# mahfuzalhasan/WaveFormer

Hardware: AMD Instinct MI355X
Metric: 128³×4 volumes/sec fwd (1/2/4/8 MI355X) + Dice Δ vs reference (higher is better)
Workload: dtype bf16x3

## Files before the change

### include/waveformer_hip.h

```cpp
#ifndef WAVEFORMER_HIP_H
#define WAVEFORMER_HIP_H

#include <stdint.h>

#ifdef __cplusplus
extern "C" {
#endif

#define WF_ABI_VERSION 21

enum { WF_PREC_BF16 = 0, WF_PREC_BF16X3 = 1, WF_PREC_FP16 = 2 };

enum {
  WF_OK = 0,
  WF_E_SHAPE = -1,
  WF_E_NULLPTR = -2,
  WF_E_LAUNCH = -3
};

int wf_abi_version(void);
const char* wf_last_error(void);


int wf_cast_f32_to_bf16(const float* in, uint16_t* out, int64_t n, void* stream);

int wf_split_f32_to_bf16x2(const float* in, uint16_t* out, int64_t n, void* stream);

int wf_split_f32_to_bf16x2_multi(const int64_t* table_dev, int64_t n, int64_t total,
                                 void* stream);

int wf_cast_f32_to_f16x2(const float* in, uint16_t* out, int64_t n, void* stream);
int wf_cast_f32_to_f16x2_multi(const int64_t* table_dev, int64_t n, int64_t total,
                               void* stream);

int wf_debug_poison_lds(int64_t blocks, int lds_bytes, void* stream);

int wf_patch_embed_fwd(const float* x, const float* w, const float* bias, float* out,
                       int64_t B, int64_t Cin, int64_t Cout, int64_t D, int64_t H, int64_t W,
                       void* stream);
int wf_patch_embed_ll_fwd(const float* x, const float* w, const float* bias, float* out,
                          const float* ln_w, const float* ln_b, float ln_eps, float* ll,
                          int64_t B, int64_t Cin, int64_t Cout, int64_t D, int64_t H, int64_t W,
// ... 159 lines not shown
int wf_window_attention_levels_fused(const int64_t* dhw, int nlev, int64_t B, int64_t C,
                                     int64_t heads, int precision);

int wf_msfuse_fwd(const float* const* src, const int64_t* src_dhw, int nsrc,
                  const float* shortcut, const float* branch_scale, float* out, float* stats,
                  float ln_eps, int64_t B, int64_t C, int64_t D, int64_t H, int64_t W,
                  void* stream);

int64_t wf_ccf_ffn_workspace_bytes(int64_t B, int64_t C, int64_t hidden, int64_t D, int64_t H,
                                   int64_t W, int precision);
int wf_ccf_ffn_fwd(const float* xh, const float* stats, const float* n2_w, const float* n2_b,
                   const uint16_t* pw_bf16x2, const float* pw_b, const float* ln1_w,
                   const float* ln1_b, float eps1, const float* dw_w, const float* dw_b,
                   const float* ln2_w, const float* ln2_b, float eps2,
                   const uint16_t* fc_bf16x2, const float* fc_b, const float* branch_scale,
                   float* out, void* workspace,
                   int64_t B, int64_t C, int64_t hidden, int64_t D, int64_t H, int64_t W,
                   int precision, void* stream);
int wf_ccf_ffn_stage(int stage, const float* xh, const float* stats, const float* n2_w,
                     const float* n2_b, const uint16_t* pw_bf16x2, const float* pw_b,
                     const float* ln1_w, const float* ln1_b, float eps1, const float* dw_w,
                     const float* dw_b, const float* ln2_w, const float* ln2_b, float eps2,
                     const uint16_t* fc_bf16x2, const float* fc_b, const float* branch_scale,
                     float* out, void* workspace, int64_t B, int64_t C, int64_t hidden,
                     int64_t D, int64_t H, int64_t W, int precision, void* stream);

int wf_patch_merging_fwd(const float* x, const float* ln_w, const float* ln_b, float eps,
                         const uint16_t* red_bf16x2, int v2, float* out, int64_t B, int64_t C,
                         int64_t D, int64_t H, int64_t W, int precision, void* stream);

int wf_proj_out_fwd(const float* x, float* out, int normalize, float eps, int64_t B,
                    int64_t C, int64_t S, void* stream);
int wf_proj_out_cl_fwd(const float* x, float* out, float eps, int64_t M, int64_t C, void* stream);

int wf_importance_map(int mode, const float* sigma_scale, float* out, int64_t rd, int64_t rh,
                      int64_t rw, void* stream);

int wf_sliding_window_stitch(const float* patches, int64_t world, int64_t slots_per_round,
                             const float* importance_map, const int64_t* starts,
                             const int64_t* nwin, float* out, int64_t B, int64_t C, int64_t D,
                             int64_t H, int64_t W, int64_t rd, int64_t rh, int64_t rw,
                             void* stream);

int wf_sliding_window_stitch_partial(const float* patches, int64_t world, int64_t rank,
                                     const float* importance_map, const int64_t* starts,
                                     const int64_t* nwin, float* out, int64_t B, int64_t C,
                                     int64_t D, int64_t H, int64_t W, int64_t rd, int64_t rh,
                                     int64_t rw, void* stream);
int wf_sliding_window_normalize(const float* num, float* out, int64_t B, int64_t C, int64_t D,
                                int64_t H, int64_t W, void* stream);

int wf_tta_merge(const float* pred, const int* flips, int npass, float* out, int64_t C,
                 int64_t D, int64_t H, int64_t W, void* stream);


int wf_window_attention_fwd_train(const float* x, const float* ln_w, const float* ln_b,
                                  float ln_eps, const uint16_t* wqkv_bf16x2, const float* bqkv,
                                  const float* bias, const uint16_t* wproj_bf16x2,
                                  const float* bproj, float* out, void* workspace, float* lse,
                                  int64_t B, int64_t C, int64_t D1, int64_t H1, int64_t W1,
                                  int64_t ws, int64_t heads, float scale, int precision,
                                  void* stream);

int64_t wf_window_attention_bwd_workspace_bytes(int64_t B, int64_t C, int64_t D1, int64_t H1,
                                                int64_t W1, int64_t ws, int64_t heads);
int wf_window_attention_bwd_core(const float* qkv, const float* o, const float* dout,
// ... 58 lines not shown
```

### waveformer_amd/_lib.py

```python
from __future__ import annotations

import ctypes
import os
import threading

_HERE = os.path.dirname(os.path.abspath(__file__))
LIB_PATH = os.environ.get("WAVEFORMER_HIP_LIB", os.path.join(_HERE, "libwaveformer_hip.so"))

_P = ctypes.c_void_p
_I64 = ctypes.c_int64
_I = ctypes.c_int
_F = ctypes.c_float

SIGNATURES = {
    "wf_abi_version": (_I, []),
    "wf_last_error": (ctypes.c_char_p, []),
    "wf_cast_f32_to_bf16": (_I, [_P, _P, _I64, _P]),
    "wf_split_f32_to_bf16x2": (_I, [_P, _P, _I64, _P]),
    "wf_split_f32_to_bf16x2_multi": (_I, [_P, _I64, _I64, _P]),
    "wf_cast_f32_to_f16x2": (_I, [_P, _P, _I64, _P]),
    "wf_cast_f32_to_f16x2_multi": (_I, [_P, _I64, _I64, _P]),
    "wf_debug_poison_lds": (_I, [_I64, _I, _P]),
    "wf_patch_embed_ll_fwd": (_I, [_P, _P, _P, _P, _P, _P, _F, _P, _I64, _I64, _I64, _I64, _I64,
                                   _I64, _P]),
# ... 40 lines not shown
    "wf_norm_act_bwd_workspace_bytes": (_I64, [_I64, _I64]),
    "wf_norm_act_bwd_cl": (_I, [_P, _I64, _P, _I64, _P, _I64, _P, _P, _I64, _P, _P, _I64, _P, _I64,
                                _I64, _I64, _I64, _F, _P, _P]),
    "wf_hf_refine_workspace_bytes": (_I64, [_I64, _I64]),
    "wf_hf_refine_fwd": (_I, [_P, _I64, _P, _P, _P, _P, _F, _P, _P, _I, _P, _P, _I64, _I64,
                              _I64, _I64, _I64, _P]),
    "wf_norm_act_cl": (_I, [_P, _I64, _P, _P, _I64, _P, _P, _I64, _I64, _I64, _I64, _F, _P]),
    "wf_upsample_trilinear_cl": (_I, [_P, _P, _I64, _I64, _I64, _I64, _I64, _I64, _I64, _I64,
                                      _I, _P]),
    "wf_linear_fwd": (_I, [_P, _P, _P, _P, _I64, _I64, _I64, _I, _I, _P]),
    "wf_window_attention_fwd_table": (_I, [_P, _P, _P, _F, _P, _P, _P, _P, _P, _P, _P,
                                           _I64, _I64, _I64, _I64, _I64, _I64, _I64, _F, _I,
                                           _P]),
    "wf_rel_pos_bias": (_I, [_P, _P, _P, _I64, _I64, _I64, _P]),
    "wf_window_attention_workspace_bytes": (_I64, [_I64, _I64, _I64, _I64, _I64, _I]),
    "wf_window_attention_fwd": (_I, [_P, _P, _P, _F, _P, _P, _P, _P, _P, _P, _P,
                                     _I64, _I64, _I64, _I64, _I64, _I64, _I64, _F, _I, _P]),
    "wf_window_attention_levels_workspace_bytes": (_I64, [_P, _I, _I64, _I64, _I]),
    "wf_window_attention_fwd_levels": (_I, [_P, _P, _I, _P, _P, _P, _P, _P, _P, _P, _I64, _I64,
                                            _I64, _F, _I, _P]),
    "wf_window_attention_fwd_levels_mode": (_I, [_P, _P, _I, _P, _P, _P, _P, _P, _P, _P, _I64,
                                                 _I64, _I64, _F, _I, _P, _I]),
    "wf_window_attention_levels_fused": (_I, [_P, _I, _I64, _I64, _I64, _I]),
    "wf_msfuse_fwd": (_I, [_P, _P, _I, _P, _P, _P, _P, _F, _I64, _I64, _I64, _I64, _I64, _P]),
    "wf_ccf_ffn_workspace_bytes": (_I64, [_I64, _I64, _I64, _I64, _I64, _I64, _I]),
    "wf_ccf_ffn_fwd": (_I, [_P, _P, _P, _P, _P, _P, _P, _P, _F, _P, _P, _P, _P, _F, _P, _P,
                            _P, _P, _P, _I64, _I64, _I64, _I64, _I64, _I64, _I, _P]),
    "wf_ccf_ffn_stage": (_I, [_I, _P, _P, _P, _P, _P, _P, _P, _P, _F, _P, _P, _P, _P, _F, _P,
                              _P, _P, _P, _P, _I64, _I64, _I64, _I64, _I64, _I64, _I, _P]),
    "wf_patch_merging_fwd": (_I, [_P, _P, _P, _F, _P, _I, _P, _I64, _I64, _I64, _I64, _I64,
                                  _I, _P]),
    "wf_proj_out_fwd": (_I, [_P, _P, _I, _F, _I64, _I64, _I64, _P]),
    "wf_proj_out_cl_fwd": (_I, [_P, _P, _F, _I64, _I64, _P]),
    "wf_upsample_dwconv3d_stats_cl": (_I, [_P, _P, _P, _P, _P] + [_I64] * 8 + [_I, _P]),
    "wf_importance_map": (_I, [_I, _P, _P, _I64, _I64, _I64, _P]),
    "wf_sliding_window_stitch": (_I, [_P, _I64, _I64, _P, _P, _P, _P, _I64, _I64, _I64, _I64,
                                      _I64, _I64, _I64, _I64, _P]),
    "wf_tta_merge": (_I, [_P, _P, _I, _P, _I64, _I64, _I64, _I64, _P]),
    "wf_sliding_window_stitch_partial": (_I, [_P, _I64, _I64, _P, _P, _P, _P, _I64, _I64,
                                              _I64, _I64, _I64, _I64, _I64, _I64, _P]),
    "wf_sliding_window_normalize": (_I, [_P, _P, _I64, _I64, _I64, _I64, _I64, _P]),
    "wf_window_attention_fwd_train": (_I, [_P, _P, _P, _F, _P, _P, _P, _P, _P, _P, _P, _P,
                                           _I64, _I64, _I64, _I64, _I64, _I64, _I64, _F, _I,
                                           _P]),
    "wf_window_attention_bwd_workspace_bytes": (_I64, [_I64, _I64, _I64, _I64, _I64, _I64,
                                                       _I64]),
    "wf_window_attention_bwd_core": (_I, [_P, _P, _P, _P, _P, _P, _P, _P, _I64, _I64, _I64,
                                          _I64, _I64, _I64, _I64, _F, _P]),
    "wf_rel_pos_bias_bwd": (_I, [_P, _P, _P, _P, _I64, _I64, _I64, _P]),
    "wf_gemm_tn_workspace_bytes": (_I64, [_I64, _I64, _I64]),
    "wf_gemm_tn": (_I, [_P, _I64, _P, _I64, _P, _I64, _I, _P, _I64, _I64, _I64, _P]),
    "wf_colsum_parts": (_I64, [_I64]),
    "wf_colsum": (_I, [_P, _I64, _I64, _P, _I64, _P, _P, _P]),
    "wf_ln_act_fwd": (_I, [_P, _P, _P, _F, _I, _P, _I64, _I64, _P]),
    "wf_ln_bwd_workspace_floats": (_I64, [_I64, _I64]),
    "wf_ln_act_bwd": (_I, [_P, _P, _P, _F, _I, _P, _P, _P, _P, _P, _P, _I64, _I64, _P]),
    "wf_dwt3d_haar_bwd": (_I, [_P, _P, _P, _I64, _I64, _I64, _I64, _I64, _P]),
    "wf_haar_analysis_ncdhw": (_I, [_P, _I64, _I64, _P, _P, _P, _I64, _I64, _I64, _I64, _I64,
                                    _P]),
    "wf_interp_adjoint_axis": (_I, [_P, _P, _I64, _I64, _I64, _I64, _P, _I64, _P]),
    "wf_interp_adjoint_axis_ac": (_I, [_P, _P, _I64, _I64, _I64, _I64, _P]),
    "wf_dwconv3d_cl": (_I, [_P, _P, _P, _I, _P, _I64, _I64, _I64, _I64, _I64, _P]),
    "wf_dwconv_wgrad_ws_floats": (_I64, [_I64] * 5),
    "wf_dwconv3d_wgrad": (_I, [_P, _P, _P, _P, _I64, _I64, _I64, _I64, _I64, _P]),
    "wf_patch_merging_gather": (_I, [_P, _I, _P, _I64, _I64, _I64, _I64, _I64, _P]),
    "wf_patch_merging_scatter": (_I, [_P, _I, _P, _I64, _I64, _I64, _I64, _I64, _P]),
    "wf_patchify": (_I, [_P, _P, _I, _I64, _I64, _I64, _I64, _I64, _P]),
    "wf_transpose_cs": (_I, [_P, _P, _I64, _I64, _I64, _P]),
}

ABI_VERSION = 21
_lock = threading.Lock()
_lib = None
_err = None


class LibraryMissing(RuntimeError):
    pass


def load(path: str | None = None):
    global _lib, _err
    with _lock:
        if _lib is not None:
            return _lib
        p = path or LIB_PATH
        if not os.path.exists(p):
            _err = f"{p} not found: build it with `python -c 'import __graft_entry__ as g; g.build()'`"
            raise LibraryMissing(_err)
        lib = ctypes.CDLL(p)
        for name, (res, args) in SIGNATURES.items():
            fn = getattr(lib, name)
            fn.restype = res
            fn.argtypes = args
        ver = lib.wf_abi_version()
        if ver != ABI_VERSION:
            raise LibraryMissing(f"{p}: ABI version {ver}, expected {ABI_VERSION} (rebuild)")
        _lib = lib
        return _lib


def call(name: str, *args) -> None:
    lib = load()
    rc = getattr(lib, name)(*args)
# ... 8 lines not shown
```

### waveformer_amd/csrc/ffn.hip

```cpp
#include "kernels.hpp"

namespace wf {

template <typename T>
struct Store4;
template <>
struct Store4<uint16_t> {
  typedef bf16x4 vec;
  static __device__ __forceinline__ f32x4 up(vec u) {
    return f32x4{bf2f((uint16_t)u[0]), bf2f((uint16_t)u[1]), bf2f((uint16_t)u[2]),
                 bf2f((uint16_t)u[3])};
  }
  static __device__ __forceinline__ uint16_t down(float v) { return f2bf(v); }
  static __device__ __forceinline__ vec zero() { return vec{0, 0, 0, 0}; }
  static __device__ __forceinline__ void store4(uint16_t* p, f32x4 v) {
    bf16x4 o;
    o[0] = (short)f2bf(v.x);
    o[1] = (short)f2bf(v.y);
    o[2] = (short)f2bf(v.z);
    o[3] = (short)f2bf(v.w);
    *reinterpret_cast<bf16x4*>(p) = o;
  }
};
template <>
// ... 645 lines not shown
  f.N = (int)C;
  f.K = (int)hidden;
  f.epi = EPI_RESID;
  f.bias = fc_b;
  f.r_x = xh;
  f.r_stats = stats;
  f.r_ln_w = n2_w;
  f.r_ln_b = n2_b;
  f.r_scale = branch_scale;
  f.rows_per_sample = D * H * W;
  f.out = out;
  f.out_bf16 = 0;
  f.ldo = C;
  if (!keep) {
    f.kpart = reinterpret_cast<float*>(h1);
    f.kpart_bytes = one;
  }
  return launch_gemm(f, s, "wf_ccf_ffn_fwd(fc)");
}

extern "C" int wf_ccf_ffn_fwd(const float* xh, const float* stats, const float* n2_w,
                              const float* n2_b, const uint16_t* pw_bf16x2, const float* pw_b,
                              const float* ln1_w, const float* ln1_b, float eps1,
                              const float* dw_w, const float* dw_b, const float* ln2_w,
                              const float* ln2_b, float eps2, const uint16_t* fc_bf16x2,
                              const float* fc_b, const float* branch_scale, float* out,
                              void* workspace, int64_t B, int64_t C, int64_t hidden, int64_t D,
                              int64_t H, int64_t W, int precision, void* stream) {
  return wf_ccf_ffn_stage(0, xh, stats, n2_w, n2_b, pw_bf16x2, pw_b, ln1_w, ln1_b, eps1, dw_w,
                          dw_b, ln2_w, ln2_b, eps2, fc_bf16x2, fc_b, branch_scale, out,
                          workspace, B, C, hidden, D, H, W, precision, stream);
}

extern "C" int wf_patch_merging_fwd(const float* x, const float* ln_w, const float* ln_b,
                                    float eps, const uint16_t* red_bf16x2, int v2, float* out,
                                    int64_t B, int64_t C, int64_t D, int64_t H, int64_t W,
                                    int precision, void* stream) {
  WF_REQUIRE(B >= 1 && C % 8 == 0 && C >= 8, "C must be a positive multiple of 8");
  WF_REQUIRE(D % 2 == 0 && H % 2 == 0 && W % 2 == 0 && D >= 2 && H >= 2 && W >= 2,
             "odd sizes (the F.pad branch, wave_helper.py:180-182) are not supported");
  WF_REQUIRE(valid_prec(precision), "unknown precision");
  WF_REQUIRE_PTR(x);
  WF_REQUIRE_PTR(ln_w);
  WF_REQUIRE_PTR(ln_b);
  WF_REQUIRE_PTR(red_bf16x2);
  WF_REQUIRE_PTR(out);
  GemmArgs g{};
  g.prec = precision;
  g.a_src = x;
  g.a_bf16 = 0;
  g.a_C = (int)C;
  g.a_nseg = 8;
  g.a_map = MAP_MERGE;
  g.merge_code = v2 ? 0x76543210 : 0x71251240;
  g.mB = (int)B;
  g.mD = (int)D;
  g.mH = (int)H;
  g.mW = (int)W;
  g.a_ln = LN_COMPUTE;
  g.a_ln_w = ln_w;
  g.a_ln_b = ln_b;
  g.a_eps = eps;
  g.w = red_bf16x2;
  g.M = B * (D / 2) * (H / 2) * (W / 2);
  g.N = (int)(2 * C);
  g.K = (int)(8 * C);
  g.epi = EPI_STORE;
  g.bias = nullptr;
  g.out = out;
  g.out_bf16 = 0;
  g.ldo = 2 * C;
  if (try_launch_merge_resident(g, (hipStream_t)stream)) return check_launch("wf_patch_merging_fwd");
  return launch_gemm(g, (hipStream_t)stream, "wf_patch_merging_fwd");
}
```

### waveformer_amd/csrc/kernels.hpp

```cpp
#pragma once
#include "wf_common.hpp"

namespace wf {

enum Prec { PREC_BF16 = 0, PREC_SPLIT = 1, PREC_FP16 = 2 };

typedef _Float16 f16x4 __attribute__((ext_vector_type(4)));
typedef _Float16 f16x8 __attribute__((ext_vector_type(8)));
__device__ __forceinline__ uint16_t f2h(float f) { return __builtin_bit_cast(uint16_t, (_Float16)f); }

template <int P>
__device__ __forceinline__ uint16_t op_cvt(float x) {
  if constexpr (P == PREC_FP16) return f2h(x);
  else return f2bf(x);
}
template <int P>
__device__ __forceinline__ short op_lo(float x, uint16_t hi) {
  if constexpr (P == PREC_SPLIT) return (short)f2bf(x - bf2f(hi));
  else return (short)0;
}
template <int P>
__device__ __forceinline__ f32x4 mma32(bf16x8 a, bf16x8 b, f32x4 c) {
  if constexpr (P == PREC_FP16)
    return __builtin_amdgcn_mfma_f32_16x16x32_f16(__builtin_bit_cast(f16x8, a),
// ... 92 lines not shown
  int64_t rows_per_sample;
  float* o_pstats;
  float* kpart;
  int64_t kpart_bytes;
  int ksplit;
  const float* lv_src[WF_MAX_LEVELS];
  int lv_row0[WF_MAX_LEVELS];
  int lv_D[WF_MAX_LEVELS], lv_H[WF_MAX_LEVELS], lv_W[WF_MAX_LEVELS];
};

int launch_gemm(const GemmArgs& g, hipStream_t s, const char* who);
int gemm_kc_pick_nt(const GemmArgs& g);
int launch_instnorm_partial(const float* x, int64_t ldx, int64_t B, int64_t C, int64_t P,
                            double* acc, hipStream_t s);
int try_launch_gemm_rows(const GemmArgs& g, hipStream_t s, bool single_chunk_only);

int launch_attn_core(const void* qkv, const float* bias, void* out, float* lse, int64_t Bw,
                     int N, int heads, int hd, float scale, int prec, hipStream_t s,
                     int table_ws = 0, int64_t pair_windows = -1, const GemmArgs* fused = nullptr);
bool attn_tbl_pair_loop(int64_t wh);

int launch_dwconv_ln_gelu(const void* in, const float* w, const float* b, const float* ln_w,
                          const float* ln_b, float eps, void* out, int B, int Hd, int D, int H,
                          int W, int prec, hipStream_t s);
int launch_dwconv3d(const void* in, const float* w, const float* b, void* out, float* pstats,
                    int B, int Hd, int D, int H, int W, int prec, hipStream_t s,
                    double* cstats = nullptr, const float* ln1_stats = nullptr,
                    const float* ln1_w = nullptr, const float* ln1_b = nullptr, int flip = 0);
int launch_ln_stats_finalize(const float* pstats, int np, int group, float eps, float* out,
                             int64_t M, hipStream_t s);
constexpr int DW_STAT_GROUP = 32;
int try_launch_gemm_kc(const GemmArgs& g, hipStream_t s);
int try_launch_merge_resident(const GemmArgs& g, hipStream_t s);
int try_launch_pw2_resident(const GemmArgs& g, hipStream_t s);
int try_launch_gemm_lnw(const GemmArgs& g, hipStream_t s);
bool gemm_lnw_wide_shape(const GemmArgs& g);

}

#include "ffn_dwfc_common.hpp"
```

### waveformer_amd/csrc/merge.hip

```cpp
#include <algorithm>

#include "gemm_common.hpp"

namespace wf {

constexpr int MR_C = 48;
constexpr int MR_K = 8 * MR_C;
constexpr int MR_N = 2 * MR_C;
constexpr int MR_NT = MR_N / 16;
constexpr int MR_KS = MR_K / 32;
constexpr int MR_KP = MR_K + WF_LDS_KPAD;
constexpr int MR_WAVES = 8;

template <int P>
__global__ __launch_bounds__(64 * MR_WAVES, 1) void merge_res_kernel(GemmArgs g) {
  constexpr bool SPLIT = P == PREC_SPLIT;
  constexpr int NPL = SPLIT ? 2 : 1;
  extern __shared__ __attribute__((aligned(16))) uint16_t Wl[];
  float* lnw = reinterpret_cast<float*>(Wl + NPL * MR_N * MR_KP);
  float* lnb = lnw + MR_K;
  const int tid = threadIdx.x, lane = tid & 63, wid = tid >> 6;
  const int l15 = lane & 15, g4 = lane >> 4;

  constexpr int OCT = MR_K / 8;
  for (int it = tid; it < NPL * MR_N * OCT; it += 64 * MR_WAVES) {
    const int pr = it / OCT, ch = it - pr * OCT;
    *reinterpret_cast<bf16x8*>(Wl + pr * MR_KP + 8 * ch) =
        *reinterpret_cast<const bf16x8*>(g.w + (int64_t)pr * MR_K + 8 * ch);
  }
  for (int i = tid; i < MR_K; i += 64 * MR_WAVES) {
    lnw[i] = g.a_ln_w[i];
    lnb[i] = g.a_ln_b[i];
  }
  __syncthreads();

  const int M = (int)g.M;
  const int ntiles = (M + 15) >> 4;
  const int hd = g.mD >> 1, hh = g.mH >> 1, hw = g.mW >> 1;
  for (int tile = blockIdx.x * MR_WAVES + wid; tile < ntiles; tile += gridDim.x * MR_WAVES) {
    const int row = tile * 16 + l15;
    int r = min(row, M - 1);
    const int x = r % hw;
    r /= hw;
    const int y = r % hh;
    r /= hh;
    const int z = r % hd, b = r / hd;
    const float* src = reinterpret_cast<const float*>(g.a_src) +
                       (int64_t)(((b * g.mD + 2 * z) * g.mH + 2 * y) * g.mW + 2 * x) * MR_C;
    int g4o = g4;
    asm volatile("" : "+v"(g4o));
    int koff[MR_KS];
#pragma unroll
    for (int ks = 0; ks < MR_KS; ++ks) {
      const int k = ks * 32 + 8 * g4o;
      const int seg = k / MR_C, c = k - seg * MR_C;
      const int o = (g.merge_code >> (4 * seg)) & 0xF;
      koff[ks] = ((((o >> 2) & 1) * g.mH + ((o >> 1) & 1)) * g.mW + (o & 1)) * MR_C + c;
    }
    float a[MR_KS][8];
#pragma unroll
    for (int ks = 0; ks < MR_KS; ++ks) {
      const f32x4* p = reinterpret_cast<const f32x4*>(src + koff[ks]);
      const f32x4 u0 = p[0], u1 = p[1];
      a[ks][0] = u0.x; a[ks][1] = u0.y; a[ks][2] = u0.z; a[ks][3] = u0.w;
      a[ks][4] = u1.x; a[ks][5] = u1.y; a[ks][6] = u1.z; a[ks][7] = u1.w;
    }
    const float sh = __shfl(a[0][0], l15, 64);
    float s = 0.f, q = 0.f;
    asm volatile("" : "+v"(q));
#pragma unroll
    for (int ks = 0; ks < MR_KS; ++ks)
#pragma unroll
      for (int j = 0; j < 8; ++j) {
        const float d = a[ks][j] - sh;
        s += d;
        q += d * d;
      }
    s = xsum16(s);
    s = xsum32(s);
    q = xsum16(q);
    q = xsum32(q);
    const float kf = (float)g.K;
    const float ms = s / kf;
    const float mean = sh + ms;
    const float rstd = rsqrtf(fmaxf(q / kf - ms * ms, 0.f) + g.a_eps);

    uint32_t wb = (uint32_t)((l15 * MR_KP + 8 * g4) * 2), lb = (uint32_t)(8 * g4 * 4);
    asm volatile("" : "+v"(wb), "+v"(lb));
    const char* Wb = reinterpret_cast<const char*>(Wl) + wb;
    const char* Lw = reinterpret_cast<const char*>(lnw) + lb;
    const char* Lb = reinterpret_cast<const char*>(lnb) + lb;
    f32x4 acc[MR_NT];
#pragma unroll
    for (int t = 0; t < MR_NT; ++t) acc[t] = f32x4{0.f, 0.f, 0.f, 0.f};
#pragma unroll
    for (int ks = 0; ks < MR_KS; ++ks) {
      __builtin_amdgcn_sched_barrier(0);
      bf16x8 ah, al;
      a_fragment<P>(a[ks], mean, rstd, reinterpret_cast<const float*>(Lw),
                    reinterpret_cast<const float*>(Lb), ks * 32, true, true, false, ah, al);
#pragma unroll
      for (int t = 0; t < MR_NT; ++t) {
        const int wo = (t * 16 * MR_KP + ks * 32) * 2;
        const bf16x8 bh = *reinterpret_cast<const bf16x8*>(Wb + wo);
        const bf16x8 bl = SPLIT ? *reinterpret_cast<const bf16x8*>(Wb + MR_N * MR_KP * 2 + wo) : bh;
        acc[t] = mma3<P>(acc[t], bh, bl, ah, al);
        if (t % 3 == 2) __builtin_amdgcn_sched_barrier(0);
      }
    }
    if (row < M) {
      float* o = reinterpret_cast<float*>(g.out) + (int64_t)row * g.ldo + 4 * g4;
#pragma unroll
      for (int t = 0; t < MR_NT; ++t) *reinterpret_cast<f32x4*>(o + 16 * t) = acc[t];
    }
  }
}

int try_launch_merge_resident(const GemmArgs& g, hipStream_t s) {
  static const bool off = getenv("WF_MERGE_RES") != nullptr && getenv("WF_MERGE_RES")[0] == '0';
  if (off || g.a_map != MAP_MERGE || g.a_C != MR_C || g.K != MR_K || g.N != MR_N ||
      g.a_ln != LN_COMPUTE || g.a_bf16 || g.out_bf16 || g.epi != EPI_STORE || g.bias ||
      g.o_pstats || g.ldo < MR_N || (g.prec != PREC_SPLIT && g.prec != PREC_FP16) || g.M < 1 ||
      g.M >= ((int64_t)1 << 31) - 16)
    return 0;
  const bool split = g.prec == PREC_SPLIT;
  const size_t lds = (size_t)(split ? 2 : 1) * MR_N * MR_KP * 2 + (size_t)2 * MR_K * 4;
  void (*kern)(GemmArgs) = split ? merge_res_kernel<PREC_SPLIT> : merge_res_kernel<PREC_FP16>;
  set_max_lds(reinterpret_cast<const void*>(kern), (int)lds);
  const int64_t ntiles = (g.M + 15) / 16;
  const unsigned gx = (unsigned)std::min<int64_t>(cdiv(ntiles, MR_WAVES), 256);
  hipLaunchKernelGGL(kern, dim3(gx), dim3(64 * MR_WAVES), lds, s, g);
  return 1;
}

}
```

### waveformer_amd/network_models/waveformer.py

```python
from __future__ import annotations

import math
import time
from typing import List, Tuple

import torch
import torch.nn as nn
import torch.nn.init as init

from .. import autograd as wfa
from .. import ops
from ..blocks import PatchEmbed as _MonaiPatchEmbed
from . import wave_helper as WH
from .wave_helper import Block, PatchMerging


class MultiscaleTransformer(nn.Module):
    def __init__(self, img_size=(128, 128, 128), patch_size=2, in_chans=4, num_classes=4,
                 embed_dims=[48, 96, 192, 384], num_heads=[3, 6, 12, 24], mlp_ratios=[4, 4, 4, 4],
                 decom_levels=[3, 2, 1, 0], multi_scale_attention=True, qkv_bias=False,
                 qk_scale=None, drop_rate=0., attn_drop_rate=0., drop_path_rate=0.,
                 norm_layer=nn.LayerNorm, patch_norm=False, depths=[2, 2, 2, 2],
                 network_config=None):
        super().__init__()
# ... 59 lines not shown
    def load_dualpath_model(self, model: nn.Module, model_file):
        t0 = time.time()
        if isinstance(model_file, str):
            sd = torch.load(model_file, map_location=torch.device('cpu'), weights_only=True)
            if 'model' in sd.keys():
                sd = sd['model']
        else:
            sd = model_file
        model.load_state_dict(sd, strict=False)
        if hasattr(self, 'logger'):
            self.logger.info(f"Load model, Time usage: {time.time() - t0}")

    def forward_features(self, x_rgb: torch.Tensor, normalize: bool = True, *,
                         channel_last: bool = False) -> Tuple[List[torch.Tensor], List]:
        if self.patch_norm:
            raise NotImplementedError("waveformer_amd: patch_norm=True is not implemented")
        if x_rgb.dtype != torch.float32:
            raise TypeError("waveformer_amd: float32 input expected")
        pe = self.patch_embed.proj
        train = wfa.needs_grad(x_rgb, *self.parameters())
        ll0 = None
        b0 = self.block1[0]
        if train:
            x = wfa.PatchEmbedFn.apply(x_rgb.contiguous(), pe.weight.contiguous(), pe.bias)
        elif (len(self.block1) > 1 and b0.ms_attention and b0.level > 0
              and x_rgb.is_cuda and not torch.compiler.is_compiling()):
            r = ops.patch_embed_ll(x_rgb.contiguous(), pe.weight.contiguous(), pe.bias,
                                   (b0.norm1.weight, b0.norm1.bias, b0.norm1.eps))
            x, ll0 = r if r is not None else (
                ops.patch_embed(x_rgb.contiguous(), pe.weight.contiguous(), pe.bias), None)
        else:
            x = ops.patch_embed(x_rgb.contiguous(), pe.weight.contiguous(), pe.bias)
        outs, outs_hf = [], []
        for s in range(4):
            if s > 0:
                x = getattr(self, f"downsample_{s}")(x)
            x_h = None
            blocks = getattr(self, f"block{s + 1}")
            for i, blk in enumerate(blocks):
                skip = not train and i < len(blocks) - 1
                WH.HF_SKIP.blocks = {id(blk): ll0 if s == 0 and i == 0 else None} if skip else {}
                try:
                    r = blk(x)
                finally:
                    WH.HF_SKIP.blocks = {}
                if isinstance(r, tuple):
                    x, x_h = r
                else:
                    x = r
            B, D, H, W, C = x.shape
            if train:
                outs.append(wfa.ProjOutFn.apply(x, bool(normalize), 1e-5))
            elif channel_last:
                outs.append(ops.proj_out_cl(x, normalize))
            else:
                outs.append(ops.proj_out(x, normalize))
            if s < 3:
                outs_hf.append(x_h if x_h is not None else ())
        return outs, outs_hf

    def forward(self, x_rgb: torch.Tensor, *, channel_last: bool = False):
        with ops.weight_scope(self):
            return self.forward_features(x_rgb, channel_last=channel_last)

    def flops(self) -> int:
        return 0
```

### waveformer_amd/ops.py

```python
from __future__ import annotations

import ctypes
import math
import os
import threading
import weakref
from typing import Dict, List, Optional, Sequence, Tuple

import torch

from . import _lib

DETAIL_KEYS = ("aad", "ada", "add", "daa", "dad", "dda", "ddd")


def _stream() -> int:
    return torch.cuda.current_stream().cuda_stream


def _ptr(t: Optional[torch.Tensor]) -> Optional[int]:
    return None if t is None else t.data_ptr()


def _check(t: torch.Tensor, name: str, dtype=torch.float32, contiguous=True) -> None:
# ... 1385 lines not shown


def tta_merge(pred: torch.Tensor, passes: Sequence[Sequence[int]]) -> torch.Tensor:
    _check(pred, "pred")
    P, C, D, H, W = pred.shape
    if len(passes) != P:
        raise ValueError(f"tta_merge: {len(passes)} passes for {P} predictions")
    masks = [sum(1 << (d - 2) for d in f) for f in passes]
    out = torch.empty((1, C, D, H, W), dtype=torch.float32, device=pred.device)
    _lib.call("wf_tta_merge", pred.data_ptr(), (ctypes.c_int * P)(*masks), P, out.data_ptr(),
              C, D, H, W, _stream())
    return out


def proj_out(x_cl: torch.Tensor, normalize: bool, eps: float = 1e-5) -> torch.Tensor:
    _check(x_cl, "x")
    B, D, H, W, C = x_cl.shape
    out = torch.empty((B, C, D, H, W), dtype=torch.float32, device=x_cl.device)
    _lib.call("wf_proj_out_fwd", x_cl.data_ptr(), out.data_ptr(), int(bool(normalize)),
              float(eps), B, C, D * H * W, _stream())
    return out


def proj_out_cl(x_cl: torch.Tensor, normalize: bool, eps: float = 1e-5) -> torch.Tensor:
    _check(x_cl, "x")
    B, D, H, W, C = x_cl.shape
    out = torch.empty_like(x_cl)
    if normalize:
        _lib.call("wf_proj_out_cl_fwd", x_cl.data_ptr(), out.data_ptr(), float(eps),
                  B * D * H * W, C, _stream())
    else:
        out.copy_(x_cl)
    return out.permute(0, 4, 1, 2, 3)
```

Baseline: 1320.

## Fuse stage-0 output projection into the patch-merging resident kernel

Adds a stage-exit kernel that, while loading the stage-0 activations for patch merging, also computes the per-voxel layer-norm and writes the stage-0 output, either NCDHW or channel-last. The separate proj_out pass over the largest activation tensor goes away, since the data is read once for both uses. Sub-lattices that the merge code never names are loaded as extra rows so the projection still covers every voxel. The cost is extra register pressure and cross-lane permlane exchanges inside the resident merge kernel, which may reduce its throughput.

```diff
diff --git a/include/waveformer_hip.h b/include/waveformer_hip.h
--- a/include/waveformer_hip.h
+++ b/include/waveformer_hip.h
@@ -7,7 +7,7 @@
 extern "C" {
 #endif
 
-#define WF_ABI_VERSION 21
+#define WF_ABI_VERSION 22
 
 enum { WF_PREC_BF16 = 0, WF_PREC_BF16X3 = 1, WF_PREC_FP16 = 2 };
 
@@ -233,6 +233,12 @@
 int wf_proj_out_fwd(const float* x, float* out, int normalize, float eps, int64_t B,
                     int64_t C, int64_t S, void* stream);
 int wf_proj_out_cl_fwd(const float* x, float* out, float eps, int64_t M, int64_t C, void* stream);
+int wf_stage_exit_taken(int64_t B, int64_t C, int64_t D, int64_t H, int64_t W, int v2,
+                        int precision);
+int wf_stage_exit_fwd(const float* x, const float* ln_w, const float* ln_b, float eps,
+                      const uint16_t* red_bf16x2, int v2, float* merged_out, float* proj_out,
+                      int normalize, float proj_eps, int channel_last, int64_t B, int64_t C,
+                      int64_t D, int64_t H, int64_t W, int precision, void* stream);
 
 int wf_importance_map(int mode, const float* sigma_scale, float* out, int64_t rd, int64_t rh,
                       int64_t rw, void* stream);
diff --git a/waveformer_amd/_lib.py b/waveformer_amd/_lib.py
--- a/waveformer_amd/_lib.py
+++ b/waveformer_amd/_lib.py
@@ -96,6 +96,9 @@
                                   _I, _P]),
     "wf_proj_out_fwd": (_I, [_P, _P, _I, _F, _I64, _I64, _I64, _P]),
     "wf_proj_out_cl_fwd": (_I, [_P, _P, _F, _I64, _I64, _P]),
+    "wf_stage_exit_taken": (_I, [_I64, _I64, _I64, _I64, _I64, _I, _I]),
+    "wf_stage_exit_fwd": (_I, [_P, _P, _P, _F, _P, _I, _P, _P, _I, _F, _I, _I64, _I64, _I64,
+                               _I64, _I64, _I, _P]),
     "wf_upsample_dwconv3d_stats_cl": (_I, [_P, _P, _P, _P, _P] + [_I64] * 8 + [_I, _P]),
     "wf_importance_map": (_I, [_I, _P, _P, _I64, _I64, _I64, _P]),
     "wf_sliding_window_stitch": (_I, [_P, _I64, _I64, _P, _P, _P, _P, _I64, _I64, _I64, _I64,
@@ -133,7 +136,7 @@
     "wf_transpose_cs": (_I, [_P, _P, _I64, _I64, _I64, _P]),
 }
 
-ABI_VERSION = 21
+ABI_VERSION = 22
 _lock = threading.Lock()
 _lib = None
 _err = None
diff --git a/waveformer_amd/csrc/ffn.hip b/waveformer_amd/csrc/ffn.hip
--- a/waveformer_amd/csrc/ffn.hip
+++ b/waveformer_amd/csrc/ffn.hip
@@ -701,19 +701,10 @@
                           workspace, B, C, hidden, D, H, W, precision, stream);
 }
 
-extern "C" int wf_patch_merging_fwd(const float* x, const float* ln_w, const float* ln_b,
-                                    float eps, const uint16_t* red_bf16x2, int v2, float* out,
-                                    int64_t B, int64_t C, int64_t D, int64_t H, int64_t W,
-                                    int precision, void* stream) {
-  WF_REQUIRE(B >= 1 && C % 8 == 0 && C >= 8, "C must be a positive multiple of 8");
-  WF_REQUIRE(D % 2 == 0 && H % 2 == 0 && W % 2 == 0 && D >= 2 && H >= 2 && W >= 2,
-             "odd sizes (the F.pad branch, wave_helper.py:180-182) are not supported");
-  WF_REQUIRE(valid_prec(precision), "unknown precision");
-  WF_REQUIRE_PTR(x);
-  WF_REQUIRE_PTR(ln_w);
-  WF_REQUIRE_PTR(ln_b);
-  WF_REQUIRE_PTR(red_bf16x2);
-  WF_REQUIRE_PTR(out);
+static GemmArgs patch_merging_args(const float* x, const float* ln_w, const float* ln_b,
+                                   float eps, const uint16_t* red_bf16x2, int v2, float* out,
+                                   int64_t B, int64_t C, int64_t D, int64_t H, int64_t W,
+                                   int precision) {
   GemmArgs g{};
   g.prec = precision;
   g.a_src = x;
@@ -721,7 +712,7 @@
   g.a_C = (int)C;
   g.a_nseg = 8;
   g.a_map = MAP_MERGE;
-  g.merge_code = v2 ? 0x76543210 : 0x71251240;
+  g.merge_code = (int)(v2 ? MERGE_CODE_V2 : MERGE_CODE_Q3);
   g.mB = (int)B;
   g.mD = (int)D;
   g.mH = (int)H;
@@ -739,6 +730,58 @@
   g.out = out;
   g.out_bf16 = 0;
   g.ldo = 2 * C;
+  return g;
+}
+
+static bool patch_merging_shape(int64_t B, int64_t C, int64_t D, int64_t H, int64_t W) {
+  return B >= 1 && C % 8 == 0 && C >= 8 && D % 2 == 0 && H % 2 == 0 && W % 2 == 0 && D >= 2 &&
+         H >= 2 && W >= 2;
+}
+
+extern "C" int wf_patch_merging_fwd(const float* x, const float* ln_w, const float* ln_b,
+                                    float eps, const uint16_t* red_bf16x2, int v2, float* out,
+                                    int64_t B, int64_t C, int64_t D, int64_t H, int64_t W,
+                                    int precision, void* stream) {
+  WF_REQUIRE(B >= 1 && C % 8 == 0 && C >= 8, "C must be a positive multiple of 8");
+  WF_REQUIRE(D % 2 == 0 && H % 2 == 0 && W % 2 == 0 && D >= 2 && H >= 2 && W >= 2,
+             "odd sizes (the F.pad branch, wave_helper.py:180-182) are not supported");
+  WF_REQUIRE(valid_prec(precision), "unknown precision");
+  WF_REQUIRE_PTR(x);
+  WF_REQUIRE_PTR(ln_w);
+  WF_REQUIRE_PTR(ln_b);
+  WF_REQUIRE_PTR(red_bf16x2);
+  WF_REQUIRE_PTR(out);
+  const GemmArgs g = patch_merging_args(x, ln_w, ln_b, eps, red_bf16x2, v2, out, B, C, D, H, W,
+                                        precision);
   if (try_launch_merge_resident(g, (hipStream_t)stream)) return check_launch("wf_patch_merging_fwd");
   return launch_gemm(g, (hipStream_t)stream, "wf_patch_merging_fwd");
 }
+
+extern "C" int wf_stage_exit_taken(int64_t B, int64_t C, int64_t D, int64_t H, int64_t W, int v2,
+                                   int precision) {
+  if (!valid_prec(precision) || !patch_merging_shape(B, C, D, H, W)) return 0;
+  const GemmArgs g = patch_merging_args(nullptr, nullptr, nullptr, 0.f, nullptr, v2, nullptr, B,
+                                        C, D, H, W, precision);
+  return try_launch_merge_exit(g, nullptr, 0, 0.f, 0, true, nullptr);
+}
+
+extern "C" int wf_stage_exit_fwd(const float* x, const float* ln_w, const float* ln_b, float eps,
+                                 const uint16_t* red_bf16x2, int v2, float* merged_out,
+                                 float* proj_out, int normalize, float proj_eps,
+                                 int channel_last, int64_t B, int64_t C, int64_t D, int64_t H,
+                                 int64_t W, int precision, void* stream) {
+  WF_REQUIRE(wf_stage_exit_taken(B, C, D, H, W, v2, precision),
+             "not a stage-exit shape (wf_stage_exit_taken): run wf_patch_merging_fwd and "
+             "wf_proj_out_fwd");
+  WF_REQUIRE_PTR(x);
+  WF_REQUIRE_PTR(ln_w);
+  WF_REQUIRE_PTR(ln_b);
+  WF_REQUIRE_PTR(red_bf16x2);
+  WF_REQUIRE_PTR(merged_out);
+  WF_REQUIRE_PTR(proj_out);
+  const GemmArgs g = patch_merging_args(x, ln_w, ln_b, eps, red_bf16x2, v2, merged_out, B, C, D,
+                                        H, W, precision);
+  try_launch_merge_exit(g, proj_out, normalize, proj_eps, channel_last, false,
+                        (hipStream_t)stream);
+  return check_launch("wf_stage_exit_fwd");
+}
diff --git a/waveformer_amd/csrc/kernels.hpp b/waveformer_amd/csrc/kernels.hpp
--- a/waveformer_amd/csrc/kernels.hpp
+++ b/waveformer_amd/csrc/kernels.hpp
@@ -148,6 +148,9 @@
 constexpr int DW_STAT_GROUP = 32;
 int try_launch_gemm_kc(const GemmArgs& g, hipStream_t s);
 int try_launch_merge_resident(const GemmArgs& g, hipStream_t s);
+constexpr unsigned MERGE_CODE_Q3 = 0x71251240u, MERGE_CODE_V2 = 0x76543210u;
+int try_launch_merge_exit(const GemmArgs& g, float* proj, int normalize, float proj_eps,
+                          int channel_last, bool dry, hipStream_t s);
 int try_launch_pw2_resident(const GemmArgs& g, hipStream_t s);
 int try_launch_gemm_lnw(const GemmArgs& g, hipStream_t s);
 bool gemm_lnw_wide_shape(const GemmArgs& g);
diff --git a/waveformer_amd/csrc/merge.hip b/waveformer_amd/csrc/merge.hip
--- a/waveformer_amd/csrc/merge.hip
+++ b/waveformer_amd/csrc/merge.hip
@@ -12,9 +12,79 @@
 constexpr int MR_KP = MR_K + WF_LDS_KPAD;
 constexpr int MR_WAVES = 8;
 
-template <int P>
-__global__ __launch_bounds__(64 * MR_WAVES, 1) void merge_res_kernel(GemmArgs g) {
+struct ExitArgs {
+  float* proj;
+  int normalize;
+  float eps;
+};
+struct NoExit {};
+
+enum ExitLayout { EXIT_NONE = 0, EXIT_NCDHW = 1, EXIT_CL = 2 };
+
+__device__ __forceinline__ void oct_sums(const float (&v)[8], float (&c)[2]) {
+  c[0] = (v[0] + v[1]) + (v[2] + v[3]);
+  c[1] = (v[4] + v[5]) + (v[6] + v[7]);
+}
+__device__ __forceinline__ void oct_sqdevs(const float (&v)[8], float m, float (&c)[2]) {
+#pragma clang fp contract(off)
+  float d[8];
+#pragma unroll
+  for (int j = 0; j < 8; ++j) d[j] = v[j] - m;
+  c[0] = fmaf(d[0], d[0], d[1] * d[1]) + fmaf(d[2], d[2], d[3] * d[3]);
+  c[1] = fmaf(d[4], d[4], d[5] * d[5]) + fmaf(d[6], d[6], d[7] * d[7]);
+}
+__device__ __forceinline__ float xchg32(float v, bool hi) {
+  const auto t = __builtin_amdgcn_permlane32_swap(__float_as_uint(v), __float_as_uint(v), true, false);
+  return __uint_as_float(hi ? t[0] : t[1]);
+}
+__device__ __forceinline__ float own_row_total(const float (&c0)[2], const float (&c1)[2],
+                                               const float (&c2)[2], bool hi) {
+  float p[2];
+#pragma unroll
+  for (int k = 0; k < 2; ++k) {
+    const float first = hi ? c1[k] : c0[k], third = hi ? c2[k] : c1[k];
+    const float mid = xchg32(hi ? c0[k] : c2[k], hi);
+    p[k] = (first + mid) + third;
+  }
+  return xsum16(p[0] + p[1]);
+}
+__device__ __forceinline__ void xchg32(const float (&p)[8], const float (&q)[8], bool hi,
+                                       float (&r)[8]) {
+#pragma unroll
+  for (int j = 0; j < 8; ++j) {
+    const auto t = __builtin_amdgcn_permlane32_swap(__float_as_uint(p[j]), __float_as_uint(q[j]),
+                                                    true, false);
+    r[j] = __uint_as_float(hi ? t[0] : t[1]);
+  }
+}
+
+constexpr int mc_missing(unsigned code, int i) {
+  int n = 0;
+  for (int o = 0; o < 8; ++o) {
+    bool seen = false;
+    for (int s = 0; s < 8; ++s) seen |= (int)((code >> (4 * s)) & 7) == o;
+    if (!seen && n++ == i) return o;
+  }
+  return -1;
+}
+constexpr int mc_nmissing(unsigned code) {
+  int n = 0;
+  while (mc_missing(code, n) >= 0) ++n;
+  return n;
+}
+constexpr int mc_row_of(unsigned code, int o) {
+  for (int s = 0; s < 8; ++s)
+    if ((int)((code >> (4 * s)) & 7) == o) return s;
+  for (int i = 0; mc_missing(code, i) >= 0; ++i)
+    if (mc_missing(code, i) == o) return 8 + i;
+  return -1;
+}
+constexpr bool mc_repeat(unsigned code, int s) { return mc_row_of(code, (code >> (4 * s)) & 7) != s; }
+
+template <int P, int PX, int NX, unsigned CODE, bool NORMK, class Exit>
+__device__ __forceinline__ void merge_res_body(const GemmArgs& g, const Exit& e) {
   constexpr bool SPLIT = P == PREC_SPLIT;
+  constexpr int NOCT = MR_KS + 3 * NX / 2;
   constexpr int NPL = SPLIT ? 2 : 1;
   extern __shared__ __attribute__((aligned(16))) uint16_t Wl[];
   float* lnw = reinterpret_cast<float*>(Wl + NPL * MR_N * MR_KP);
@@ -49,21 +119,122 @@
                        (int64_t)(((b * g.mD + 2 * z) * g.mH + 2 * y) * g.mW + 2 * x) * MR_C;
     int g4o = g4;
     asm volatile("" : "+v"(g4o));
-    int koff[MR_KS];
-#pragma unroll
-    for (int ks = 0; ks < MR_KS; ++ks) {
+    int koff[NOCT];
+#pragma unroll
+    for (int ks = 0; ks < NOCT; ++ks) {
       const int k = ks * 32 + 8 * g4o;
       const int seg = k / MR_C, c = k - seg * MR_C;
-      const int o = (g.merge_code >> (4 * seg)) & 0xF;
+      int o = (g.merge_code >> (4 * seg)) & 0xF;
+      if constexpr (NX > 0)
+        if (ks >= MR_KS) o = seg == 8 ? mc_missing(CODE, 0) : mc_missing(CODE, 1);
       koff[ks] = ((((o >> 2) & 1) * g.mH + ((o >> 1) & 1)) * g.mW + (o & 1)) * MR_C + c;
     }
-    float a[MR_KS][8];
-#pragma unroll
-    for (int ks = 0; ks < MR_KS; ++ks) {
+    float a[NOCT][8];
+#pragma unroll
+    for (int ks = 0; ks < NOCT; ++ks) {
       const f32x4* p = reinterpret_cast<const f32x4*>(src + koff[ks]);
       const f32x4 u0 = p[0], u1 = p[1];
       a[ks][0] = u0.x; a[ks][1] = u0.y; a[ks][2] = u0.z; a[ks][3] = u0.w;
       a[ks][4] = u1.x; a[ks][5] = u1.y; a[ks][6] = u1.z; a[ks][7] = u1.w;
+    }
+    if constexpr (PX != EXIT_NONE) {
+      constexpr int NROW = 8 + NX;
+      const bool hi = g4 >= 2, live = row < M;
+      auto exit_phase = [&](auto NORM_) {
+#pragma clang fp contract(off)
+      constexpr bool NORM = decltype(NORM_)::value;
+      float mean[NROW], rstd[NROW];
+#pragma unroll
+      for (int m = 0; m < NROW / 2; ++m) {
+        mean[2 * m] = mean[2 * m + 1] = 0.f;
+        rstd[2 * m] = rstd[2 * m + 1] = 1.f;
+        if constexpr (NORM) {
+          __builtin_amdgcn_sched_barrier(0);
+          float c0[2], c1[2], c2[2];
+          oct_sums(a[3 * m], c0);
+          oct_sums(a[3 * m + 1], c1);
+          oct_sums(a[3 * m + 2], c2);
+          const float own_mean = own_row_total(c0, c1, c2, hi) / (float)MR_C;
+          const float oth_mean = xchg32(own_mean, hi);
+          const float mA = hi ? oth_mean : own_mean, mB = hi ? own_mean : oth_mean;
+          oct_sqdevs(a[3 * m], mA, c0);
+          oct_sqdevs(a[3 * m + 1], own_mean, c1);
+          oct_sqdevs(a[3 * m + 2], mB, c2);
+          const float own_rstd = rsqrtf(own_row_total(c0, c1, c2, hi) / (float)MR_C + e.eps);
+          const float oth_rstd = xchg32(own_rstd, hi);
+          mean[2 * m] = mA;
+          mean[2 * m + 1] = mB;
+          rstd[2 * m] = hi ? oth_rstd : own_rstd;
+          rstd[2 * m + 1] = hi ? own_rstd : oth_rstd;
+        }
+        if constexpr (PX == EXIT_CL) {
+          float* pb = e.proj + (src - reinterpret_cast<const float*>(g.a_src));
+#pragma unroll
+          for (int u = 0; u < 3; ++u) {
+            const int ks = 3 * m + u;
+            const bool second = u == 2 || (u == 1 && hi);
+            const bool dup = m < 4 && (second ? mc_repeat(CODE, (2 * m + 1) & 7) : mc_repeat(CODE, (2 * m) & 7));
+            const float mu = second ? mean[2 * m + 1] : mean[2 * m];
+            const float rs = second ? rstd[2 * m + 1] : rstd[2 * m];
+            if (!live || dup) continue;
+            float v[8];
+#pragma unroll
+            for (int j = 0; j < 8; ++j) v[j] = NORM ? (a[ks][j] - mu) * rs : a[ks][j];
+            f32x4* p = reinterpret_cast<f32x4*>(pb + koff[ks]);
+            p[0] = f32x4{v[0], v[1], v[2], v[3]};
+            p[1] = f32x4{v[4], v[5], v[6], v[7]};
+          }
+        }
+      }
+      if constexpr (PX == EXIT_NCDHW) {
+        static_assert(NX == mc_nmissing(CODE), "NX: the sub-lattices CODE never names");
+        const int64_t S = (int64_t)g.mD * g.mH * g.mW;
+        float* pb = e.proj + (int64_t)b * MR_C * S + ((int64_t)(2 * z) * g.mH + 2 * y) * g.mW + 2 * x;
+        auto pair = [&](auto Q) {
+          constexpr int q = decltype(Q)::value;
+          __builtin_amdgcn_sched_barrier(0);
+          constexpr int s0 = mc_row_of(CODE, 2 * q), s1 = mc_row_of(CODE, 2 * q + 1);
+          constexpr int m0 = s0 >> 1, m1 = s1 >> 1;
+          constexpr bool odd0 = s0 & 1, odd1 = s1 & 1;
+          float* pq = pb + ((q >> 1) * g.mH + (q & 1)) * g.mW;
+          const float mu0 = mean[s0], rs0 = rstd[s0], mu1 = mean[s1], rs1 = rstd[s1];
+          auto store = [&](const float(&v0)[8], const float(&v1)[8], int j, bool on) {
+            float* p = pq + (int64_t)(8 * j) * S;
+            if (!on) return;
+#pragma unroll
+            for (int i = 0; i < 8; ++i) {
+              f32x2 o = {v0[i], v1[i]};
+              if constexpr (NORM) o = f32x2{(v0[i] - mu0) * rs0, (v1[i] - mu1) * rs1};
+              *reinterpret_cast<f32x2*>(p + (int64_t)i * S) = o;
+            }
+          };
+          float ra[8], rb[8];
+          if constexpr (odd0 == odd1) {
+            constexpr int ua = odd0 ? 2 : 0;
+            store(a[3 * m0 + ua], a[3 * m1 + ua], g4 + ua, live);
+            store(a[3 * m0 + 1], a[3 * m1 + 1], odd0 ? g4 - 2 : g4 + 4, live && hi == odd0);
+          } else if constexpr (!odd0) {
+            xchg32(a[3 * m1 + 1], a[3 * m1 + 2], hi, ra);
+            xchg32(a[3 * m1 + 2], a[3 * m1 + 2], hi, rb);
+            store(a[3 * m0], ra, g4, live);
+            store(a[3 * m0 + 1], rb, g4 + 4, live && !hi);
+          } else {
+            xchg32(a[3 * m1], a[3 * m1], hi, ra);
+            xchg32(a[3 * m1 + 1], a[3 * m1 + 1], hi, rb);
+            float f[8];
+#pragma unroll
+            for (int i = 0; i < 8; ++i) f[i] = hi ? a[3 * m0 + 1][i] : a[3 * m0 + 2][i];
+            store(f, ra, hi ? g4 - 2 : g4 + 2, live);
+            store(a[3 * m0 + 2], rb, g4 + 2, live && hi);
+          }
+        };
+        pair(std::integral_constant<int, 0>{});
+        pair(std::integral_constant<int, 1>{});
+        pair(std::integral_constant<int, 2>{});
+        pair(std::integral_constant<int, 3>{});
+      }
+      };
+      exit_phase(std::integral_constant<bool, NORMK>{});
     }
     const float sh = __shfl(a[0][0], l15, 64);
     float s = 0.f, q = 0.f;
@@ -116,21 +287,69 @@
   }
 }
 
+template <int P>
+__global__ __launch_bounds__(64 * MR_WAVES, 1) void merge_res_kernel(GemmArgs g) {
+  merge_res_body<P, EXIT_NONE, 0, 0u, false>(g, NoExit{});
+}
+
+template <int P, int PX, unsigned CODE, bool NORMK>
+__global__ __launch_bounds__(64 * MR_WAVES, 1) void merge_exit_kernel(GemmArgs g, ExitArgs e) {
+  merge_res_body<P, PX, mc_nmissing(CODE), CODE, NORMK>(g, e);
+}
+
+static bool merge_resident_shape(const GemmArgs& g) {
+  static const bool off = getenv("WF_MERGE_RES") != nullptr && getenv("WF_MERGE_RES")[0] == '0';
+  return !(off || g.a_map != MAP_MERGE || g.a_C != MR_C || g.K != MR_K || g.N != MR_N ||
+           g.a_ln != LN_COMPUTE || g.a_bf16 || g.out_bf16 || g.epi != EPI_STORE || g.bias ||
+           g.o_pstats || g.ldo < MR_N || (g.prec != PREC_SPLIT && g.prec != PREC_FP16) ||
+           g.M < 1 || g.M >= ((int64_t)1 << 31) - 16);
+}
+static size_t merge_resident_lds(bool split) {
+  return (size_t)(split ? 2 : 1) * MR_N * MR_KP * 2 + (size_t)2 * MR_K * 4;
+}
+static unsigned merge_resident_grid(const GemmArgs& g) {
+  const int64_t ntiles = (g.M + 15) / 16;
+  return (unsigned)std::min<int64_t>(cdiv(ntiles, MR_WAVES), 256);
+}
+
 int try_launch_merge_resident(const GemmArgs& g, hipStream_t s) {
-  static const bool off = getenv("WF_MERGE_RES") != nullptr && getenv("WF_MERGE_RES")[0] == '0';
-  if (off || g.a_map != MAP_MERGE || g.a_C != MR_C || g.K != MR_K || g.N != MR_N ||
-      g.a_ln != LN_COMPUTE || g.a_bf16 || g.out_bf16 || g.epi != EPI_STORE || g.bias ||
-      g.o_pstats || g.ldo < MR_N || (g.prec != PREC_SPLIT && g.prec != PREC_FP16) || g.M < 1 ||
-      g.M >= ((int64_t)1 << 31) - 16)
-    return 0;
+  if (!merge_resident_shape(g)) return 0;
   const bool split = g.prec == PREC_SPLIT;
-  const size_t lds = (size_t)(split ? 2 : 1) * MR_N * MR_KP * 2 + (size_t)2 * MR_K * 4;
+  const size_t lds = merge_resident_lds(split);
   void (*kern)(GemmArgs) = split ? merge_res_kernel<PREC_SPLIT> : merge_res_kernel<PREC_FP16>;
   set_max_lds(reinterpret_cast<const void*>(kern), (int)lds);
-  const int64_t ntiles = (g.M + 15) / 16;
-  const unsigned gx = (unsigned)std::min<int64_t>(cdiv(ntiles, MR_WAVES), 256);
-  hipLaunchKernelGGL(kern, dim3(gx), dim3(64 * MR_WAVES), lds, s, g);
+  hipLaunchKernelGGL(kern, dim3(merge_resident_grid(g)), dim3(64 * MR_WAVES), lds, s, g);
   return 1;
 }
 
-}
+int try_launch_merge_exit(const GemmArgs& g, float* proj, int normalize, float proj_eps,
+                          int channel_last, bool dry, hipStream_t s) {
+  ExitArgs e{proj, normalize, proj_eps};
+  const bool v2 = (unsigned)g.merge_code == MERGE_CODE_V2;
+  if (!merge_resident_shape(g) || (!v2 && (unsigned)g.merge_code != MERGE_CODE_Q3))
+    return 0;
+  if (dry) return 1;
+  const bool split = g.prec == PREC_SPLIT;
+  const size_t lds = merge_resident_lds(split);
+  auto launch = [&](auto kern) {
+    set_max_lds(reinterpret_cast<const void*>(kern), (int)lds);
+    hipLaunchKernelGGL(kern, dim3(merge_resident_grid(g)), dim3(64 * MR_WAVES), lds, s, g, e);
+  };
+  auto by_layout = [&](auto P_, auto CODE_) {
+    constexpr int P = decltype(P_)::value;
+    constexpr unsigned CODE = decltype(CODE_)::value;
+    if (channel_last && normalize) launch(merge_exit_kernel<P, EXIT_CL, CODE, true>);
+    else if (channel_last) launch(merge_exit_kernel<P, EXIT_CL, CODE, false>);
+    else if (normalize) launch(merge_exit_kernel<P, EXIT_NCDHW, CODE, true>);
+    else launch(merge_exit_kernel<P, EXIT_NCDHW, CODE, false>);
+  };
+  auto by_code = [&](auto P_) {
+    if (v2) by_layout(P_, std::integral_constant<unsigned, MERGE_CODE_V2>{});
+    else by_layout(P_, std::integral_constant<unsigned, MERGE_CODE_Q3>{});
+  };
+  if (split) by_code(std::integral_constant<int, PREC_SPLIT>{});
+  else by_code(std::integral_constant<int, PREC_FP16>{});
+  return 1;
+}
+
+}
diff --git a/waveformer_amd/network_models/waveformer.py b/waveformer_amd/network_models/waveformer.py
--- a/waveformer_amd/network_models/waveformer.py
+++ b/waveformer_amd/network_models/waveformer.py
@@ -115,8 +115,11 @@
         else:
             x = ops.patch_embed(x_rgb.contiguous(), pe.weight.contiguous(), pe.bias)
         outs, outs_hf = [], []
+        merged = None
         for s in range(4):
-            if s > 0:
+            if merged is not None:
+                x, merged = merged, None
+            elif s > 0:
                 x = getattr(self, f"downsample_{s}")(x)
             x_h = None
             blocks = getattr(self, f"block{s + 1}")
@@ -132,7 +135,16 @@
                 else:
                     x = r
             B, D, H, W, C = x.shape
-            if train:
+            r = None
+            ds = self.downsample_1
+            if (s == 0 and not train and x.is_cuda and not torch.compiler.is_compiling()
+                    and isinstance(ds, WH.PatchMergingV2)):
+                r = ops.stage_exit(x.contiguous(), ds.norm, ds.reduction, ds._v2, normalize,
+                                   channel_last)
+            if r is not None:
+                proj, merged = r
+                outs.append(proj)
+            elif train:
                 outs.append(wfa.ProjOutFn.apply(x, bool(normalize), 1e-5))
             elif channel_last:
                 outs.append(ops.proj_out_cl(x, normalize))
diff --git a/waveformer_amd/ops.py b/waveformer_amd/ops.py
--- a/waveformer_amd/ops.py
+++ b/waveformer_amd/ops.py
@@ -1441,3 +1441,33 @@
     else:
         out.copy_(x_cl)
     return out.permute(0, 4, 1, 2, 3)
+
+
+def stage_exit(x_cl: torch.Tensor, norm: torch.nn.LayerNorm, reduction: torch.nn.Linear,
+               v2: bool, normalize: bool, channel_last: bool = False, eps: float = 1e-5
+               ) -> Optional[Tuple[torch.Tensor, torch.Tensor]]:
+    return _stage_exit_raw(x_cl, norm.weight, norm.bias, float(norm.eps), reduction.weight, v2,
+                           normalize, channel_last, eps, _prec())
+
+
+def _stage_exit_raw(x_cl, ln_w, ln_b, ln_eps, red_w, v2, normalize, channel_last, eps, prec
+                    ) -> Optional[Tuple[torch.Tensor, torch.Tensor]]:
+    B, D, H, W, C = x_cl.shape
+    if (tuple(red_w.shape) != (2 * C, 8 * C) or ln_w.numel() != 8 * C or ln_b.numel() != 8 * C
+            or not _lib.query("wf_stage_exit_taken", B, C, D, H, W, int(bool(v2)), prec)):
+        return None
+    _check(x_cl, "x")
+    _check(ln_w, "ln_w")
+    _check(ln_b, "ln_b")
+    red = split_weight(red_w, prec=prec)
+    merged = torch.empty((B, D // 2, H // 2, W // 2, 2 * C), dtype=torch.float32,
+                         device=x_cl.device)
+    if channel_last:
+        proj = torch.empty_like(x_cl)
+    else:
+        proj = torch.empty((B, C, D, H, W), dtype=torch.float32, device=x_cl.device)
+    _lib.call("wf_stage_exit_fwd", x_cl.data_ptr(), ln_w.data_ptr(), ln_b.data_ptr(),
+              float(ln_eps), red.data_ptr(), int(bool(v2)), merged.data_ptr(), proj.data_ptr(),
+              int(bool(normalize)), float(eps), int(bool(channel_last)), B, C, D, H, W, prec,
+              _stream())
+    return (proj.permute(0, 4, 1, 2, 3) if channel_last else proj), merged
```

New measurement: 1291. -2.2%, worse.
